# turtle-robotics/sea-current

Measured on AMD Instinct MI355X. Metric: plans/sec (batched start-goal, 1024^2 grid), higher is better.
Workload: dtype int32; 1 GPU; 1024x1024 random-obstacle grids (salt20, one grid and one query block per step), EDT + A*, 1024 batched queries per GPU and step, 10 steps = 10240 queries per library call; queries_per_launch=10240, map=salt20, queries_per_gpu=1024, queries_total=1024, lmax=4096, parallelism=query-sharded x1, contexts_in_flight=2, steps_per_call=10, hw_queues=4

## Files before the change

### sea-current_amd/csrc/astar.hip

```cpp
#include "sc_internal.h"
#include <stdlib.h>

#define NBUCKET 32
#define ASTAR_CQ_THROUGHPUT 1024
#define ASTAR_RU_THROUGHPUT 4
#define ASTAR_CQ_LATENCY 2048
#define ASTAR_RU_LATENCY 8
#define E_RUN (1u << 18)
#define E_START (4u << 13 | 3u << 16)
#define RUNK 8

struct astar_args {
    const uint8_t* moves;
    const int32_t* d2;
    int W, H;
    int32_t rmin;
    const int32_t* start;
    const int32_t* goal;
    const int32_t* qgrid;
    const int32_t* order;
    const int32_t* nq_dev;
    int nq;
    int Lmax;
    int32_t* path;
    int32_t* len;
    int32_t* cost;
    int32_t* status;
    void* g;
    uint32_t* closed;
    uint32_t* buckets;
    int cap;
    int32_t* expanded;
    int32_t* counter;
    int32_t* ovf_list;
    int32_t* ovf_count;
    int32_t* ovf_sticky;
    int nstat;
    int lazy;
    int tw, bw;
    size_t gcells, bwords;
};

__device__ __forceinline__ int octile(int x, int y, int gx, int gy) {
    int dx = abs(x - gx), dy = abs(y - gy);
    return 10 * max(dx, dy) + 4 * min(dx, dy);
}

__device__ __forceinline__ uint32_t gix(int x, int y, int tw) {
    return ((((uint32_t)(y >> 2) * (uint32_t)tw + (uint32_t)(x >> 2)) << 4) | ((uint32_t)(y & 3) << 2)) | (uint32_t)(x & 3);
}
__device__ __forceinline__ uint32_t gix8(int x, int y, int tw8) {
    return ((((uint32_t)(y >> 3) * (uint32_t)tw8 + (uint32_t)(x >> 3)) << 6) | ((uint32_t)(y & 7) << 3)) | (uint32_t)(x & 7);
}
template <typename GT> __device__ __forceinline__ uint32_t gidx(int x, int y, int tw);
template <> __device__ __forceinline__ uint32_t gidx<uint32_t>(int x, int y, int tw) { return gix(x, y, tw); }
template <> __device__ __forceinline__ uint32_t gidx<uint8_t>(int x, int y, int tw) { return gix8(x, y, tw); }
__device__ __forceinline__ uint32_t cix(int x, int y, int bw) {
    return (((uint32_t)(y >> 4) * (uint32_t)bw + (uint32_t)(x >> 5)) << 4) | (uint32_t)(y & 15);
}

template <typename T>
__device__ __forceinline__ T g_load(const T* p) {
    return __hip_atomic_load(p, __ATOMIC_RELAXED, __HIP_MEMORY_SCOPE_AGENT);
}

__device__ __forceinline__ uint32_t prune_always(int d) {
    const unsigned long long T = 0x75B6D9EA34C851A2ull;
    return (uint32_t)(T >> (8 * d)) & 0xFFu;
}

__device__ __forceinline__ uint32_t entry_pack(int x, int y, int d, uint32_t pmv) {
    const int e0 = (int)((0x6476u >> (4 * (d & 3))) & 7u), e1 = (int)((0x7554u >> (4 * (d & 3))) & 7u);
    const uint32_t side = d < 4 ? (((pmv >> e0) & 1u) | (((pmv >> e1) & 1u) << 1)) : 0u;
    return (uint32_t)y << 19 | side << 16 | (uint32_t)d << 13 | (uint32_t)x;
}
__device__ __forceinline__ uint32_t entry_prune(uint32_t e) {
    const int d = (int)((e >> 13) & 7u);
    uint32_t prune = prune_always(d);
    const int k0 = d < 2 ? 3 : 0, k1 = d < 2 ? 2 : 1;
    const int e0 = (int)((0x6476u >> (4 * (d & 3))) & 7u), e1 = (int)((0x7554u >> (4 * (d & 3))) & 7u);
    if ((e >> 16) & 1u) prune |= (1u << k0) | (1u << e0);
    if ((e >> 17) & 1u) prune |= (1u << k1) | (1u << e1);
    if (e & E_RUN) prune |= 1u << d;
    return (e & 0x3E000u) == E_START ? 0u : prune;
}
// ... 67 lines not shown
}

__device__ __forceinline__ uint32_t bcast_group8(uint32_t v) {
    const uint32_t q = (uint32_t)__builtin_amdgcn_update_dpp(0, (int)v, 0x00 , 0xF, 0xF, false);
    const uint32_t r = (uint32_t)__builtin_amdgcn_update_dpp(0, (int)q, 0x114 , 0xF, 0xF, false);
    return q | r;
}

#define HQ 256
#define ASTAR_SPIN_LIMIT (1 << 20)
template <typename GT, bool DUAL, int CQ, int REFILL_UNROLL>
__device__ __forceinline__ void astar_query(const astar_args& a, const int q, const int slot) {
    constexpr int REFILL = CQ / 2;
    __shared__ uint32_t qe[CQ + 64];
    __shared__ int s_head[NBUCKET];
    __shared__ int s_tail[NBUCKET];
    __shared__ uint32_t nd_xy[64];
    __shared__ uint32_t nd_mv[64];
    __shared__ uint16_t succ[512];
    __shared__ uint8_t prune_tbl[64];
    __shared__ uint32_t dup_tbl[DUAL ? 1024 + 64 : 1];
    __shared__ uint2 hq_rec[DUAL ? HQ + 64 : 1];
    __shared__ int hq_tail, hq_head, hq_clean, hq_stop, hq_ovf, hq_fcur, hq_found, hq_flush;
    constexpr int SCOPE = DUAL ? __HIP_MEMORY_SCOPE_WORKGROUP : __HIP_MEMORY_SCOPE_WAVEFRONT;
    const int lane = threadIdx.x & 63;
    const int wv = DUAL ? __builtin_amdgcn_readfirstlane((int)(threadIdx.x >> 6)) : 0;
    const int W = a.W, H = a.H;
    const size_t cells = (size_t)W * H;
    const int s = a.start[q], t = a.goal[q];
    int32_t* path = a.path + (size_t)q * a.Lmax;

    int out_st = SC_Q_OK, out_len = 0, out_cost = -1, nexp = 0, npop = 0, kcyc = 0, nstep = 0;
    const size_t grid_off = a.qgrid ? (size_t)a.qgrid[q] * cells : 0;
    const uint8_t* const mvs = a.moves + grid_off;
    const bool bad = s < 0 || t < 0 || (size_t)s >= cells || (size_t)t >= cells || a.d2[grid_off + s] < a.rmin || a.d2[grid_off + t] < a.rmin;
    if (bad) out_st = SC_Q_BAD_ENDPOINT;
    else if (s == t) {
        if (lane == 0 && wv == 0) path[0] = s;
        out_len = 1; out_cost = 0; nexp = 1;
    } else {
    const int tw = a.tw, bw = a.bw;
    GT* g = static_cast<GT*>(a.g) + (size_t)slot * a.gcells;
    uint32_t* cl = a.closed + (size_t)slot * a.bwords;
    uint32_t* bk = a.buckets + (size_t)slot * NBUCKET * a.cap;
    const int cap = a.cap, capm = a.cap - 1;
    const int sx = s % W, sy = s / W, gx = t % W, gy = t / W;
    const int ddx[8] = {1, -1, 0, 0, 1, -1, 1, -1};
    const int ddy[8] = {0, 0, 1, -1, 1, 1, -1, -1};

    {
        uint4* p = reinterpret_cast<uint4*>(cl);
        const size_t n4 = a.bwords >> 2;
        for (size_t i = DUAL ? threadIdx.x : lane; i < n4; i += DUAL ? 128 : 64) p[i] = make_uint4(0, 0, 0, 0);
    }
    __builtin_amdgcn_wave_barrier();
    if (wv == 0 && lane < NBUCKET) { s_head[lane] = 0; s_tail[lane] = 0; }
    if (wv == 0) prune_tbl[lane] = (uint8_t)entry_prune((uint32_t)lane << 13);
    if (DUAL)
        for (int i = threadIdx.x; i < 1024 + 64; i += 128) dup_tbl[i] = 0xFFFFFFFFu;
    int fcur = octile(sx, sy, gx, gy);
    if (wv == 0 && lane == 0) {
        qe[0] = (uint32_t)sy << 19 | E_START | (uint32_t)sx;
        hq_tail = 0; hq_head = 0; hq_clean = 0; hq_stop = 0; hq_ovf = 0; hq_fcur = fcur; hq_found = 0; hq_flush = 0;
    }
    asm volatile("s_waitcnt vmcnt(0)" ::: "memory");
    wave_lds_sync();
    if (DUAL) __syncthreads();
    int lh = 0, lt = 1;

    bool found = false, ovf = false;
    const unsigned long long t_begin = __builtin_amdgcn_s_memtime();
    int steps_left = (int)(8 * cells + 1024 < 0x7FFFFFFF ? 8 * cells + 1024 : 0x7FFFFFFF);

    const int mdx = (int)((0x2252u >> (2 * (lane & 7))) & 3u) - 1;
    const int mdy = (int)((0x0A25u >> (2 * (lane & 7))) & 3u) - 1;
    const uint32_t mw = (lane & 7) < 4 ? 10u : 14u;
    const int moff = mdy * W + mdx;

    auto push_entry = [&](const bool act, const uint32_t ne, const int df) {
        const bool same = act && df == 0;
        const unsigned long long m0 = __ballot(same);
        bool spill = false;
        if (m0) {
            const int cnt = __popcll(m0);
            if (__builtin_expect(lt - lh + cnt <= CQ, 1)) {
                if (same) {
                    const int rank = __builtin_amdgcn_mbcnt_hi((uint32_t)(m0 >> 32), __builtin_amdgcn_mbcnt_lo((uint32_t)m0, 0u));
                    qe[(lt + rank) & (CQ - 1)] = ne;
                }
                lt += cnt;
            } else spill = true;
        }
        if (act && (df != 0 || spill)) {
            const int bb = (fcur + df) & 31;
            const int pos = __hip_atomic_fetch_add(&s_tail[bb], 1, __ATOMIC_RELAXED, SCOPE);
            if (__builtin_expect(pos - __hip_atomic_load(&s_head[bb], __ATOMIC_RELAXED, SCOPE) >= cap, 0)) ovf = true;
            else bk[(size_t)bb * cap + (pos & capm)] = ne;
        }
        lt = __builtin_amdgcn_readfirstlane(lt);
    };
    int hq_tl = 0, hq_hd = 0;
    auto hand_over = [&](const bool rec, const int hx, const int hy, const uint32_t hm, const uint32_t hp) {
        const unsigned long long wm = __ballot(rec);
        if (wm) {
            const int cnt = __popcll(wm);
            int waited = 0;
            while (__builtin_expect(hq_tl + cnt - hq_hd > HQ, 0)) {
                hq_hd = __builtin_amdgcn_readfirstlane(__hip_atomic_load(&hq_head, __ATOMIC_RELAXED, SCOPE));
                if (hq_tl + cnt - hq_hd > HQ) {
                    __builtin_amdgcn_s_sleep(1);
// ... 127 lines not shown
                const int n = min(tl - hd, REFILL);
                for (int base = lane; base < n; base += 64 * REFILL_UNROLL) {
                    uint32_t chunk[REFILL_UNROLL];
#pragma unroll
                    for (int k = 0; k < REFILL_UNROLL; ++k)
                        if (base + 64 * k < n) chunk[k] = bq[(hd + base + 64 * k) & capm];
#pragma unroll
                    for (int k = 0; k < REFILL_UNROLL; ++k)
                        if (base + 64 * k < n) qe[(lt + base + 64 * k) & (CQ - 1)] = chunk[k];
                }
                lt += n;
                if (lane == 0) __hip_atomic_store(&s_head[b], hd + n, __ATOMIC_RELAXED, SCOPE);
                wave_lds_sync();
            }
            const int n = min(64, lt - lh);
            npop += n; ++nstep;
            if (DUAL && n <= 16) {
                const int kl = n <= 4 ? 3 : n <= 8 ? 2 : n <= 16 ? 1 : 0, KL = 1 << kl, GL = 2 * KL;
                const int sub = lane >> (kl + 1), j = (lane >> kl) & 1, k = lane & (KL - 1);
                const bool valid = sub < n;
                const uint32_t e_raw = qe[(lh + sub) & (CQ - 1)];
                const uint32_t e = valid ? e_raw : 0u;
                lh += n;
                const int x = e & 0x1FFF, y = e >> 19;
                const uint32_t bit = 1u << (x & 31);
                const int dxg = gx - x, dyg = gy - y, adx = abs(dxg), ady = abs(dyg);
                const int dD = 4 + ((dxg < 0 ? 1 : 0) | (dyg < 0 ? 2 : 0));
                const int dS = adx > ady ? (dxg < 0 ? 1 : 0) : (dyg < 0 ? 3 : 2);
                const uint32_t bD = adx >= 1 && ady >= 1 ? 1u << dD : 0u, bS = adx != ady ? 1u << dS : 0u;
                const int d = j ? dS : dD;
                const bool has = valid && (j ? bS : bD) != 0u;
                const int lgeom = j ? abs(adx - ady) : min(adx, ady);
                const int ddx_ = (int)((0x2252u >> (2 * d)) & 3u) - 1, ddy_ = (int)((0x0A25u >> (2 * d)) & 3u) - 1;
                const uint8_t* const addr = mvs + (y * W + x) + (has ? min(k, lgeom - 1) : 0) * (ddy_ * W + ddx_);
                const bool head = valid && j == 0 && k == 0;
                uint32_t old, byte;
                uint32_t* const wa = &cl[cix(x, y, bw)];
                pop_loads_issue(addr, wa, byte, old);
                const uint32_t prune = prune_tbl[(e >> 13) & 63u];
                const int dup = dup_settle(head, x, y, e);
                pop_loads_wait(byte, old);
                const bool link = has && k < lgeom && ((byte >> d) & 1u) && (k > 0 || !((prune >> d) & 1u));
                const unsigned long long lm = __ballot(link);
                const uint32_t grp = (uint32_t)(lm >> (lane & ~(KL - 1))) & ((1u << KL) - 1u);
                const int run = __ffs((int)~grp) - 1;
                const uint32_t ne = entry_pack(x + (k + 1) * ddx_, y + (k + 1) * ddy_, d, byte) | (k + 1 < run ? E_RUN : 0u);
                const bool won1 = head && dup == 0 && !(old & bit);
                masked_or_noret(wa, won1 ? bit : 0u);
                const unsigned long long wm1 = __ballot(won1);
                const bool act = ((wm1 >> (lane & ~(GL - 1))) & 1ull) && k < run;
                {
                    const unsigned long long ma = __ballot(act);
                    if (ma) {
                        const int c = __popcll(ma);
                        if (__builtin_expect(lt - lh + c <= CQ, 1)) {
                            qe[act ? ((lt + (int)__builtin_amdgcn_mbcnt_hi((uint32_t)(ma >> 32), __builtin_amdgcn_mbcnt_lo((uint32_t)ma, 0u))) & (CQ - 1)) : CQ + lane] = ne;
                            lt += c;
                        } else push_entry(act, ne, 0);
                    }
                }
                hand_over(won1, x, y, (byte & ~prune) & ~(bD | bS), byte);
                nexp += __popcll(wm1);
            } else if (!DUAL && n <= 8) {
                const int sub = lane >> 3, d = lane & 7;
                const bool valid = sub < n;
                const uint32_t e = valid ? qe[(lh + sub) & (CQ - 1)] : 0u;
                lh += n;
                const int x = e & 0x1FFF, y = e >> 19;
                const uint32_t bit = 1u << (x & 31);
                uint32_t old = 0, pmv;
                const int hc = octile(x, y, gx, gy);
                const int nx = x + mdx, ny = y + mdy;
                const int df = (int)mw + octile(nx, ny, gx, gy) - hc;
                const int adx = abs(gx - x), ady = abs(gy - y);
                const int lgeom = d >= 4 ? min(adx, ady) : abs(adx - ady);
                const int lmax = valid && df == 0 ? min(RUNK, lgeom) : 1;
                const uint8_t* const cell = mvs + (y * W + x);
                const uint8_t* ra[RUNK - 1];
                uint32_t rm[RUNK - 1];
#pragma unroll
                for (int k = 1; k < RUNK; ++k) ra[k - 1] = cell + min(k, lmax - 1) * moff;
                pop_run_issue(ra, cell, &cl[cix(x, y, bw)], valid && d == 0 ? bit : 0u, rm, pmv, old);
                const uint32_t prune = prune_tbl[(e >> 13) & 63u];
                pop_run_wait_loads(rm, pmv, old);
                const bool cand = valid && (((pmv & ~prune) >> d) & 1u);
                int run = cand ? 1 : 0;
#pragma unroll
                for (int k = 1; k < RUNK; ++k)
                    if (run == k && k < lmax && ((rm[k - 1] >> d) & 1u)) run = k + 1;
                const uint32_t ne = entry_pack(nx, ny, d, pmv) | (run > 1 ? E_RUN : 0u);
                atomic_wait(old);
                old = bcast_group8(old);
                const bool won = valid && !(old & bit);
                push_entry(won && cand, ne, df);
#pragma unroll
                for (int k = 2; k <= RUNK; ++k) {
                    if (__ballot(won && run >= k) == 0) break;
                    push_entry(won && run >= k, entry_pack(x + k * mdx, y + k * mdy, d, rm[k - 2]) | (run > k ? E_RUN : 0u), 0);
                }
                nexp += __popcll(__ballot(won && d == 0));
                if (__ballot(won && x == gx && y == gy)) found = true;
                if (won && d == 0) g[gidx<GT>(x, y, tw)] = (GT)(fcur - hc);
            } else if (DUAL) {
                const bool valid = lane < n;
                const uint32_t e_raw = qe[(lh + lane) & (CQ - 1)];
                const uint32_t e = valid ? e_raw : 0u;
                lh += n;
                const int x = e & 0x1FFF, y = e >> 19;
                const uint32_t bit = 1u << (x & 31);
                uint32_t old, pmv;
                uint32_t* const wa = &cl[cix(x, y, bw)];
                pop_loads_issue(mvs + (y * W + x), wa, pmv, old);
                const int dup = dup_settle(valid, x, y, e);
                const uint32_t prune = prune_tbl[(e >> 13) & 63u];
                const int dxg = gx - x, dyg = gy - y, adx = abs(dxg), ady = abs(dyg);
                const int dD = 4 + ((dxg < 0 ? 1 : 0) | (dyg < 0 ? 2 : 0));
                const int dS = adx > ady ? (dxg < 0 ? 1 : 0) : (dyg < 0 ? 3 : 2);
                const uint32_t bD = adx >= 1 && ady >= 1 ? 1u << dD : 0u, bS = adx != ady ? 1u << dS : 0u;
                const int nxD = x + (dxg < 0 ? -1 : 1), nyD = y + (dyg < 0 ? -1 : 1);
                const int nxS = x + (adx > ady ? (dxg < 0 ? -1 : 1) : 0), nyS = y + (adx > ady ? 0 : (dyg < 0 ? -1 : 1));
                pop_loads_wait(pmv, old);
                const uint32_t cand = valid ? (pmv & ~prune) : 0u;
                const uint32_t neD = (uint32_t)nyD << 19 | (uint32_t)dD << 13 | (uint32_t)nxD;
                const uint32_t neS = entry_pack(nxS, nyS, dS, pmv);
                const bool won = valid && dup == 0 && !(old & bit);
                masked_or_noret(wa, won ? bit : 0u);
                {
                    const bool pD = won && (cand & bD), pS = won && (cand & bS);
                    const unsigned long long mD = __ballot(pD), mS = __ballot(pS);
                    const int cD = __popcll(mD), c2 = cD + __popcll(mS);
                    if (c2) {
                        if (__builtin_expect(lt - lh + c2 <= CQ, 1)) {
                            qe[pD ? ((lt + (int)__builtin_amdgcn_mbcnt_hi((uint32_t)(mD >> 32), __builtin_amdgcn_mbcnt_lo((uint32_t)mD, 0u))) & (CQ - 1)) : CQ + lane] = neD;
                            qe[pS ? ((lt + cD + (int)__builtin_amdgcn_mbcnt_hi((uint32_t)(mS >> 32), __builtin_amdgcn_mbcnt_lo((uint32_t)mS, 0u))) & (CQ - 1)) : CQ + lane] = neS;
                            lt += c2;
                        } else {
                            push_entry(pD, neD, 0);
                            push_entry(pS, neS, 0);
                        }
                    }
                }
                nexp += __popcll(hand_over(won, x, y, cand & ~(bD | bS), pmv));
            } else {
                const bool valid = lane < n;
                const uint32_t e = valid ? qe[(lh + lane) & (CQ - 1)] : 0u;
                lh += n;
                const int x = e & 0x1FFF, y = e >> 19;
                const uint32_t bit = 1u << (x & 31);
                uint32_t old = 0, pmv;
                pop_pair_issue(mvs + (y * W + x), &cl[cix(x, y, bw)], valid ? bit : 0u, pmv, old);
                const uint32_t prune = prune_tbl[(e >> 13) & 63u];
                const int hc = octile(x, y, gx, gy);
                pop_pair_wait_load(pmv, old);
                uint32_t mv = valid ? (pmv & ~prune) : 0u;
                nd_xy[lane] = (uint32_t)y << 16 | (uint32_t)x;
                nd_mv[lane] = pmv;
                const uint32_t cnt = (uint32_t)__popc(mv);
                int base = 0, total = 0;
#pragma unroll
                for (int bb = 0; bb < 4; ++bb) {
                    const unsigned long long m = __ballot((cnt >> bb) & 1u);
                    base += (int)__builtin_amdgcn_mbcnt_hi((uint32_t)(m >> 32), __builtin_amdgcn_mbcnt_lo((uint32_t)m, 0u)) << bb;
                    total += __popcll(m) << bb;
                }
                while (mv) {
                    const int dd = __ffs((int)mv) - 1;
                    mv &= mv - 1;
                    succ[base++] = (uint16_t)(lane << 3 | dd);
                }
                wave_lds_sync();
                bool won = false;
                for (int j0 = 0; j0 < total; j0 += 64) {
                    const bool act = j0 + lane < total;
                    const uint32_t sd = act ? succ[j0 + lane] : 0u;
                    const int par = (int)(sd >> 3), d = (int)(sd & 7u);
                    const uint32_t xy = nd_xy[par], pmvp = nd_mv[par];
                    const int px = xy & 0xFFFF, py = xy >> 16;
                    const int ddx_ = (int)((0x2252u >> (2 * d)) & 3u) - 1, ddy_ = (int)((0x0A25u >> (2 * d)) & 3u) - 1;
                    const int nx = px + ddx_, ny = py + ddy_;
                    const int df = (d < 4 ? 10 : 14) + octile(nx, ny, gx, gy) - octile(px, py, gx, gy);
                    const uint8_t* ra[RUNK - 1];
#pragma unroll
                    for (int k = 1; k < RUNK; ++k) ra[k - 1] = mvs + (py * W + px);
                    (void)ra;
                    if (j0 == 0) {
                        atomic_wait(old);
                        won = valid && !(old & bit);
                        nexp += __popcll(__ballot(won));
                        if (__ballot(won && x == gx && y == gy)) found = true;
                        nd_mv[lane] = pmv | (won ? 0x100u : 0u);
                        wave_lds_sync();
                    }
                    const bool go = act && ((nd_mv[par] >> 8) & 1u);
                    push_entry(go, entry_pack(nx, ny, d, pmvp), df);
                }
                if (total == 0) {
                    atomic_wait(old);
                    won = valid && !(old & bit);
                    nexp += __popcll(__ballot(won));
                    if (__ballot(won && x == gx && y == gy)) found = true;
                }
                if (won) g[gidx<GT>(x, y, tw)] = (GT)(fcur - hc);
            }
            lt = __builtin_amdgcn_readfirstlane(lt);
            lh = __builtin_amdgcn_readfirstlane(lh);
            nexp = __builtin_amdgcn_readfirstlane(nexp);
            found = __builtin_amdgcn_readfirstlane((int)found) != 0;
            wave_lds_sync();
            if (--steps_left < 0) ovf = true;
            if (__builtin_expect(DUAL ? steps_left < 0 : __ballot(ovf) != 0, 0)) break;
        }
        if (DUAL) {
            if (a.lazy && lane == 0) __hip_atomic_store(&hq_flush, hq_tl, __ATOMIC_RELAXED, SCOPE);
            for (int waited = 0; __builtin_amdgcn_readfirstlane(__hip_atomic_load(&hq_clean, __ATOMIC_RELAXED, SCOPE)) != hq_tl;) {
                __builtin_amdgcn_s_sleep(1);
                if (++waited > ASTAR_SPIN_LIMIT) { ovf = true; break; }
// ... 12 lines not shown
        fcur += 1 + (__ffs((int)rot) - 1);
        if (DUAL && lane == 0) __hip_atomic_store(&hq_fcur, fcur, __ATOMIC_RELAXED, SCOPE);
    }
    if (DUAL && lane == 0) __hip_atomic_store(&hq_stop, 1, __ATOMIC_RELAXED, SCOPE);
    }
    if (DUAL) __syncthreads();

    const bool overflow = __ballot(ovf) != 0;
    if (overflow) {
        if (lane == 0 && wv == 0) {
            const int i = atomicAdd(a.ovf_count, 1);
            a.ovf_list[i] = q;
            *a.ovf_sticky = 1;
        }
        out_st = SC_Q_RING_OVERFLOW;
    } else if (!found) {
        out_st = SC_Q_NO_PATH;
    } else {
        asm volatile("s_waitcnt vmcnt(0)" ::: "memory");
        const int Lmax = a.Lmax;
        int cx = gx, cy = gy, L = 1;
        uint32_t gc = (uint32_t)fcur;
        if (lane == 0) path[Lmax - 1] = t;
        bool broken = false;
        const int wox = lane % 7 - 3, woy = lane / 7 - 3;
        const int md = lane & 7;
        const int mdx_ = (int)((0x2252u >> (2 * md)) & 3u) - 1, mdy_ = (int)((0x0A25u >> (2 * md)) & 3u) - 1;
        const uint32_t mw_ = md < 4 ? 10u : 14u;
        while (!broken && (cx != sx || cy != sy)) {
            uint32_t info = 0u, gw = 0u;
            {
                const int nx = cx + wox, ny = cy + woy;
                if (lane < 49 && nx >= 0 && ny >= 0 && nx < W && ny < H) {
                    const uint32_t mvb = mvs[ny * W + nx];
                    const uint32_t cw = g_load(&cl[cix(nx, ny, bw)]);
                    gw = (uint32_t)g_load(&g[gidx<GT>(nx, ny, tw)]);
                    info = mvb | ((cw >> (nx & 31)) & 1u) << 8;
                }
            }
            int ox = 0, oy = 0;
            for (int k = 0; k < 3 && !broken && (cx != sx || cy != sy); ++k) {
                const int src = (oy - mdy_ + 3) * 7 + (ox - mdx_ + 3);
                const uint32_t ni = (uint32_t)__shfl((int)info, src, 64), ng = (uint32_t)__shfl((int)gw, src, 64);
                const bool ok = lane < 8 && ((ni >> md) & 1u) && ((ni >> 8) & 1u) && (GT)ng == (GT)(gc - mw_);
                const unsigned long long m = __ballot(ok);
                if (!m) broken = true;
                else {
                    const int d = __ffsll((long long)m) - 1;
                    cx -= ddx[d]; cy -= ddy[d];
                    ox -= ddx[d]; oy -= ddy[d];
                    gc -= (d < 4 ? 10u : 14u);
                    ++L;
                    if (lane == 0 && L <= Lmax) path[Lmax - L] = cy * W + cx;
                }
            }
        }
        if (broken) out_st = SC_Q_NO_PATH;
        else if (L > Lmax) { out_st = SC_Q_TRUNCATED; out_len = L; out_cost = fcur; }
        else {
            const int shift = Lmax - L;
            if (shift > 0) {
                __builtin_amdgcn_fence(__ATOMIC_RELEASE, "workgroup");
                for (int i = 0; i < L; i += 64) {
                    int v = 0;
                    if (i + lane < L) v = __hip_atomic_load(&path[shift + i + lane], __ATOMIC_RELAXED, __HIP_MEMORY_SCOPE_AGENT);
                    if (i + lane < L) path[i + lane] = v;
                    __builtin_amdgcn_fence(__ATOMIC_RELEASE, "workgroup");
                }
            }
            out_len = L; out_cost = fcur;
        }
    }
    kcyc = (int)((__builtin_amdgcn_s_memtime() - t_begin) >> 10);
    }
    if (lane == 0 && wv == 0) {
        a.status[q] = out_st; a.len[q] = out_len; a.cost[q] = out_cost;
        a.expanded[q] = nexp; a.expanded[a.nstat + q] = npop; a.expanded[2 * a.nstat + q] = kcyc; a.expanded[3 * a.nstat + q] = nstep;
    }
}

template <typename GT>
__global__ void __launch_bounds__(64) astar_kernel(astar_args a) {
    const int nq = a.nq_dev ? *a.nq_dev : a.nq;
    for (;;) {
        const int qi = __builtin_amdgcn_readfirstlane(atomicAdd(a.counter, 1)) >> 6;
        if (qi >= nq) break;
        astar_query<GT, false, ASTAR_CQ_THROUGHPUT, ASTAR_RU_THROUGHPUT>(a, a.order ? a.order[qi] : qi, (int)blockIdx.x);
    }
}

template <typename GT, int CQ, int RU>
__global__ void __launch_bounds__(128) astar_kernel_dual(astar_args a) {
    __shared__ int s_qi;
    const int nq = a.nq_dev ? *a.nq_dev : a.nq;
    for (;;) {
        if (threadIdx.x == 0) s_qi = atomicAdd(a.counter, 64) >> 6;
        __syncthreads();
        const int qi = __builtin_amdgcn_readfirstlane(s_qi);
        __syncthreads();
        if (qi >= nq) break;
        astar_query<GT, true, CQ, RU>(a, a.order ? a.order[qi] : qi, (int)blockIdx.x);
        __syncthreads();
    }
}

__global__ void __launch_bounds__(1024) astar_prep_kernel(const int32_t* __restrict__ start, const int32_t* __restrict__ goal, int Q, int W,
                                                          int H, int32_t* __restrict__ order, int32_t* __restrict__ ctr) {
    __shared__ int hist[1024];
    __shared__ int scan[1024];
    const int tid = threadIdx.x;
    if (tid < 4) ctr[tid] = 0;
    if (!order) return;
    hist[tid] = 0;
    __syncthreads();
    const int hmax = 14 * max(W, H) + 1;
// ... 31 lines not shown
    int per_cu = 0, dev = ctx->device;
    hipDeviceProp_t prop;
    if (hipOccupancyMaxActiveBlocksPerMultiprocessor(&per_cu, astar_kernel<uint8_t>, 64, 0) != hipSuccess || per_cu <= 0) per_cu = 8;
    if (hipGetDeviceProperties(&prop, dev) != hipSuccess || prop.multiProcessorCount <= 0) prop.multiProcessorCount = 256;
    int w = per_cu * prop.multiProcessorCount;
    if (const char* e = getenv("SC_ASTAR_WAVES")) { const int v = atoi(e); if (v > 0) w = v; }
    ctx->astar_waves = w;
    return w;
}
static int astar_resident_dual(sc_ctx* ctx, bool latency) {
    int& cached = latency ? ctx->astar_dual_lat : ctx->astar_dual;
    if (cached >= 0) return cached;
    int per_cu = 0, n = 0;
    hipDeviceProp_t prop;
    const hipError_t e_ = latency ? hipOccupancyMaxActiveBlocksPerMultiprocessor(&per_cu, astar_kernel_dual<uint8_t, ASTAR_CQ_LATENCY, ASTAR_RU_LATENCY>, 128, 0)
                                  : hipOccupancyMaxActiveBlocksPerMultiprocessor(&per_cu, astar_kernel_dual<uint8_t, ASTAR_CQ_THROUGHPUT, ASTAR_RU_THROUGHPUT>, 128, 0);
    if (e_ == hipSuccess && per_cu > 0 && hipGetDeviceProperties(&prop, ctx->device) == hipSuccess && prop.multiProcessorCount > 0)
        n = per_cu * prop.multiProcessorCount;
    if (const char* e = getenv("SC_ASTAR_DUAL")) { const int v = atoi(e); if (v == 0) n = 0; else if (v > 1 && v < n) n = v; }
    if (latency) { if (const char* e = getenv("SC_ASTAR_LATENCY")) { if (atoi(e) == 0) n = 0; } }
    cached = n;
    return n;
}

static int astar_run(sc_ctx* ctx, const int32_t* d2, int G, const int32_t* qgrid, int W, int H, int32_t r2, const int32_t* start,
                     const int32_t* goal, int Q, int Lmax, int32_t* path, int32_t* len, int32_t* cost,
                     int32_t* status, bool full_g = false) {
    const size_t cells = (size_t)W * H;
    const int tw = full_g ? (W + 3) >> 2 : (W + 7) >> 3, bw = (W + 31) >> 5;
    const size_t gcells = full_g ? (size_t)tw * ((H + 3) >> 2) * 16 : (size_t)tw * ((H + 7) >> 3) * 64;
    const size_t gsz = full_g ? 4 : 1;
    const size_t bwords = (size_t)bw * ((H + 15) >> 4) * 16;
    const int32_t rmin = r2 > 1 ? r2 : 1;
    int r = sc_scratch_reserve(ctx, &ctx->moves, cells * (size_t)G);
    if (r != SC_OK) return r;
    r = sc_launch_moves(ctx, d2, W, H * G, H, r2, (uint8_t*)ctx->moves.p);
    if (r != SC_OK) return r;
    r = sc_scratch_reserve(ctx, &ctx->qstats, (size_t)Q * 6 * sizeof(int32_t));
    if (r != SC_OK) return r;
    int32_t* expanded = (int32_t*)ctx->qstats.p;
    int32_t* order = expanded + 4 * (size_t)Q;
    int32_t* ovf_list = order + Q;
    ctx->last_Q = Q;
    int cap = ctx->astar_cap;
    if (const char* e = getenv("SC_ASTAR_CAP")) { const int v = atoi(e); if (v >= 1024 && (v & (v - 1)) == 0) cap = v; }
    if (cells > ((size_t)1 << 21)) {
        int want = 1 << 15;
        while (want < 64 * (W > H ? W : H)) want <<= 1;
        if (cap < want) cap = want;
    }
    const size_t per_slot = gcells * gsz + bwords * 4 + (size_t)NBUCKET * cap * 4;
    size_t slots = ctx->astar_slot_budget / per_slot;
    const size_t rlat = (size_t)astar_resident_dual(ctx, true);
    const bool latency = !full_g && rlat > 0 && (size_t)Q <= rlat && (size_t)Q <= slots;
    const size_t rdual = latency ? rlat : (size_t)astar_resident_dual(ctx, false);
    const bool dual = !full_g && rdual > 0;
    const size_t resident = dual ? rdual : (size_t)astar_resident_waves(ctx);
    if (slots > resident) slots = resident;
    if (slots > (size_t)Q) slots = Q;
    if (slots < 1) slots = 1;
    auto ring_slots = [](size_t n) { return n > 16 ? n : (size_t)16; };
    if (slots * gcells * gsz > ctx->gslots.bytes || slots * bwords * 4 > ctx->closed.bytes || ring_slots(slots) * NBUCKET * (size_t)cap * 4 > ctx->buckets.bytes) {
        size_t free_b = 0, total_b = 0;
        if (hipMemGetInfo(&free_b, &total_b) == hipSuccess) {
            const size_t avail = (size_t)(0.9 * (double)(free_b + ctx->gslots.bytes + ctx->closed.bytes + ctx->buckets.bytes));
            while (slots > 1 && slots * (gcells * gsz + bwords * 4) + ring_slots(slots) * NBUCKET * (size_t)cap * 4 > avail) slots = (slots + 1) / 2;
        }
    }
    for (;;) {
        r = sc_scratch_reserve(ctx, &ctx->gslots, slots * gcells * gsz);
        if (r == SC_OK) r = sc_scratch_reserve(ctx, &ctx->closed, slots * bwords * 4);
        if (r == SC_OK) r = sc_scratch_reserve(ctx, &ctx->buckets, ring_slots(slots) * NBUCKET * (size_t)cap * 4);
        if (r == SC_OK) break;
        if (r != SC_ERR_NOMEM || slots <= 1) return r;
        (void)hipGetLastError();
        slots = (slots + 1) / 2;
    }
    if (!ctx->actr.p) {
        r = sc_scratch_reserve(ctx, &ctx->actr, 16 * sizeof(int32_t));
        if (r != SC_OK) return r;
        SC_HIP(ctx, hipMemsetAsync(ctx->actr.p, 0, 16 * sizeof(int32_t), ctx->stream));
    }
    int32_t* ctr = (int32_t*)ctx->actr.p;
    ctx->status_armed = true;

    const bool sorted = (size_t)Q > slots;
    int tk = sc_time_begin(ctx, SC_K_ASTAR);
    hipLaunchKernelGGL(astar_prep_kernel, dim3(1), dim3(1024), 0, ctx->stream, start, goal, Q, W, H, sorted ? order : (int32_t*)nullptr, ctr);
    astar_args a{(const uint8_t*)ctx->moves.p, d2, W, H, rmin, start, goal, qgrid, sorted ? order : nullptr, nullptr, Q, Lmax, path, len,
                 cost, status, ctx->gslots.p, (uint32_t*)ctx->closed.p, (uint32_t*)ctx->buckets.p, cap, expanded, ctr,
                 ovf_list, ctr + 1, ctx->status + SC_ST_ASTAR_OVERFLOW, Q, (dual && (size_t)Q > slots) ? 1 : 0, tw, bw, gcells, bwords};
    if (full_g) hipLaunchKernelGGL(astar_kernel<uint32_t>, dim3((unsigned)slots), dim3(64), 0, ctx->stream, a);
    else if (dual && latency && (size_t)Q <= slots)
        hipLaunchKernelGGL((astar_kernel_dual<uint8_t, ASTAR_CQ_LATENCY, ASTAR_RU_LATENCY>), dim3((unsigned)slots), dim3(128), 0, ctx->stream, a);
    else if (dual)
        hipLaunchKernelGGL((astar_kernel_dual<uint8_t, ASTAR_CQ_THROUGHPUT, ASTAR_RU_THROUGHPUT>), dim3((unsigned)slots), dim3(128), 0, ctx->stream, a);
    else hipLaunchKernelGGL(astar_kernel<uint8_t>, dim3((unsigned)slots), dim3(64), 0, ctx->stream, a);
    {
        const size_t rslots = slots >= 16 ? slots / 16 : 1;
        const int rcap = cap * 16;
        astar_args b = a;
        b.order = ovf_list; b.nq_dev = ctr + 1; b.nq = 0; b.cap = rcap; b.counter = ctr + 2;
        b.ovf_list = order; b.ovf_count = ctr + 3;
        if (full_g) hipLaunchKernelGGL(astar_kernel<uint32_t>, dim3((unsigned)rslots), dim3(64), 0, ctx->stream, b);
        else hipLaunchKernelGGL(astar_kernel<uint8_t>, dim3((unsigned)rslots), dim3(64), 0, ctx->stream, b);
    }
    sc_time_end(ctx, tk);
    SC_HIP(ctx, hipGetLastError());
    return SC_OK;
}

extern "C" int sc_astar_batch(sc_ctx* ctx, const int32_t* d2, int W, int H, int32_t r2_clear,
                              const int32_t* start, const int32_t* goal, int Q, int Lmax,
                              int32_t* path, int32_t* len, int32_t* cost, int32_t* status) {
    if (!ctx || !d2 || !start || !goal || !path || !len || !cost || !status || W <= 0 || H <= 0 || Q < 0 ||
        Lmax <= 0 || W > SC_MAX_DIM || H > SC_MAX_DIM)
        return SC_ERR_INVALID;
    if (Q == 0) return SC_OK;
    SC_HIP(ctx, hipSetDevice(ctx->device));
    return astar_run(ctx, d2, 1, nullptr, W, H, r2_clear, start, goal, Q, Lmax, path, len, cost, status);
}

extern "C" int sc_astar_batch_multi(sc_ctx* ctx, const int32_t* d2, int G, const int32_t* qgrid, int W, int H, int32_t r2_clear,
                                    const int32_t* start, const int32_t* goal, int Q, int Lmax,
// ... 59 lines not shown
```

### sea-current_amd/csrc/moves.hip

```cpp
#include "sc_internal.h"

__global__ void __launch_bounds__(256)
moves_kernel(const int32_t* __restrict__ d2, int W, int Hall, int H, int32_t rmin, uint8_t* __restrict__ moves) {
    const int x = blockIdx.x * 256 + threadIdx.x;
    const int yall = blockIdx.y;
    if (x >= W) return;
    const int y = yall % H;
    const int32_t* r1 = d2 + (size_t)yall * W;
    bool t[3][3];
#pragma unroll
    for (int j = -1; j <= 1; ++j)
#pragma unroll
        for (int i = -1; i <= 1; ++i) {
            int xx = x + i, yy = y + j;
            t[j + 1][i + 1] = xx >= 0 && xx < W && yy >= 0 && yy < H && r1[(ptrdiff_t)j * W + xx] >= rmin;
        }
    uint32_t m = 0;
    if (t[1][1]) {
        m |= (uint32_t)t[1][2] << 0;
        m |= (uint32_t)t[1][0] << 1;
        m |= (uint32_t)t[2][1] << 2;
        m |= (uint32_t)t[0][1] << 3;
        m |= (uint32_t)(t[2][2] && t[1][2] && t[2][1]) << 4;
        m |= (uint32_t)(t[2][0] && t[1][0] && t[2][1]) << 5;
// ... 52 lines not shown
        const int32_t* r = r1 + (ptrdiff_t)(j - 1) * W;
        const int4 v = *reinterpret_cast<const int4*>(r + x);
        const int32_t l = x > 0 ? r[x - 1] : 0, q = x + 4 < W ? r[x + 4] : 0;
        t[j] = (uint32_t)(l >= rmin) | (uint32_t)(v.x >= rmin) << 1 | (uint32_t)(v.y >= rmin) << 2 | (uint32_t)(v.z >= rmin) << 3 |
               (uint32_t)(v.w >= rmin) << 4 | (uint32_t)(q >= rmin) << 5;
    }
#pragma unroll
    for (int k = 0; k < 4; ++k) {
        uint32_t out = 0;
#pragma unroll
        for (int i = 0; i < 4; ++i) {
            const uint32_t a = t[k] >> i, c = t[k + 1] >> i, b = t[k + 2] >> i;
            uint32_t m = 0;
            if (c & 2u) {
                const uint32_t E = (c >> 2) & 1u, Wt = c & 1u, S = (b >> 1) & 1u, N = (a >> 1) & 1u;
                m = E | Wt << 1 | S << 2 | N << 3 | (((b >> 2) & 1u) & E & S) << 4 | ((b & 1u) & Wt & S) << 5 | (((a >> 2) & 1u) & E & N) << 6 |
                    ((a & 1u) & Wt & N) << 7;
            }
            out |= m << (8 * i);
        }
        *reinterpret_cast<uint32_t*>(moves + (size_t)(yall0 + k) * W + x) = out;
    }
}

int sc_launch_moves(sc_ctx* ctx, const int32_t* d2, int W, int Hall, int H, int32_t r2, uint8_t* moves) {
    int32_t rmin = r2 > 1 ? r2 : 1;
    int tk = sc_time_begin(ctx, SC_K_MOVES);
    if (W % 4 == 0 && H % 4 == 0 && ((uintptr_t)d2 & 15) == 0 && ((uintptr_t)moves & 3) == 0)
        hipLaunchKernelGGL(moves4x4_kernel, dim3((W / 4 + 255) / 256, Hall / 4), dim3(256), 0, ctx->stream, d2, W, Hall, H, rmin, moves);
    else if (W % 4 == 0 && ((uintptr_t)d2 & 15) == 0 && ((uintptr_t)moves & 3) == 0)
        hipLaunchKernelGGL(moves4_kernel, dim3((W / 4 + 255) / 256, Hall), dim3(256), 0, ctx->stream, d2, W, Hall, H, rmin, moves);
    else
        hipLaunchKernelGGL(moves_kernel, dim3((W + 255) / 256, Hall), dim3(256), 0, ctx->stream, d2, W, Hall, H, rmin, moves);
    sc_time_end(ctx, tk);
    SC_HIP(ctx, hipGetLastError());
    return SC_OK;
}

extern "C" int sc_moves_i32_u8(sc_ctx* ctx, const int32_t* d2, int W, int H, int32_t r2_clear, uint8_t* moves) {
    if (!ctx || !d2 || !moves || W <= 0 || H <= 0 || W > SC_MAX_DIM || H > SC_MAX_DIM) return SC_ERR_INVALID;
    SC_HIP(ctx, hipSetDevice(ctx->device));
    return sc_launch_moves(ctx, d2, W, H, H, r2_clear, moves);
}

__host__ __device__ static inline int64_t isqrt64(int64_t v) {
    int64_t r = (int64_t)sqrt((double)v);
    while (r * r > v) --r;
    while ((r + 1) * (r + 1) <= v) ++r;
    return r;
}

__global__ void __launch_bounds__(256)
clearance_penalty_kernel(const int32_t* __restrict__ d2, size_t n, int32_t thr, int32_t r2_soft, int64_t s10, int pen_max,
                         uint8_t* __restrict__ pen) {
    const size_t i = (size_t)blockIdx.x * 256 + threadIdx.x;
    if (i >= n) return;
    const int32_t d = d2[i];
    uint8_t p = 0;
    if (d >= thr && d < r2_soft) p = (uint8_t)(((int64_t)pen_max * (s10 - isqrt64(100ll * d))) / s10);
    pen[i] = p;
}

extern "C" int sc_clearance_penalty_u8(sc_ctx* ctx, const int32_t* d2, int W, int H, int batch, int32_t r2_clear, int32_t r2_soft,
                                       int pen_max, uint8_t* pen) {
    if (!ctx || !d2 || !pen || W <= 0 || H <= 0 || W > SC_MAX_DIM || H > SC_MAX_DIM || batch <= 0 || pen_max < 0 || pen_max > 255 ||
        r2_soft < 1)
// ... 26 lines not shown
```

### sea-current_amd/csrc/sc_internal.h

```cpp
#pragma once
#include <hip/hip_runtime.h>
#include <math.h>
#include <stdint.h>
#include <stdio.h>
#include <string.h>

#include <set>
#include <vector>

#include "../../include/sea_current_hip.h"

struct sc_scratch {
    void* p = nullptr;
    size_t bytes = 0;
    sc_scratch() = default;
    sc_scratch(const sc_scratch&) = delete;
    sc_scratch& operator=(const sc_scratch&) = delete;
    ~sc_scratch() { if (p) (void)hipFree(p); }
};

static inline size_t al256(size_t b) { return (b + 255) & ~(size_t)255; }

enum sc_status_word {
    SC_ST_ASTAR_OVERFLOW,
// ... 95 lines not shown
class __attribute__((visibility("hidden"))) sc_stage {
  public:
    explicit sc_stage(sc_ctx* ctx) : ctx_(ctx) {}
    int in(const void* src, size_t bytes) {
        const int i = slot(bytes);
        if (src && bytes) up_.push_back({i, const_cast<void*>(src), bytes});
        return i;
    }
    int out(void* dst, size_t bytes) {
        const int i = slot(bytes);
        back(i, dst, bytes);
        return i;
    }
    void back(int i, void* dst, size_t bytes) {
        if (dst && bytes) down_.push_back({i, dst, bytes});
    }
    int upload();
    template <class T> T* dev(int i) const { return (T*)((char*)ctx_->host_stage.p + off_[i]); }
    int finish(int r);

  private:
    struct copy { int slot; void* host; size_t bytes; };
    int slot(size_t bytes) {
        off_.push_back(end_);
        end_ += al256(bytes ? bytes : 1);
        return (int)off_.size() - 1;
    }
    sc_ctx* ctx_;
    size_t end_ = 0;
    std::vector<size_t> off_;
    std::vector<copy> up_, down_;
};

int sc_time_begin(sc_ctx* ctx, int kid);
void sc_time_end(sc_ctx* ctx, int token);
int sc_time_chain(sc_ctx* ctx, int token, int kid);

int sc_launch_edt(sc_ctx* ctx, const uint8_t* occ, int W, int H, int batch, int32_t* d2);
int sc_launch_moves(sc_ctx* ctx, const int32_t* d2, int W, int Hall, int H, int32_t r2, uint8_t* moves);
int sc_launch_arclength(sc_ctx* ctx, const float* ctrl, int S, int nsub, float* cum, float* seg_len, const int32_t* S_dev);
int sc_launch_resample(sc_ctx* ctx, const float* ctrl, const float* cum, const float* arclength, const int32_t* seg_off, int B, int S,
                       int nsub, float* profile_pos, const int32_t* prof_off, int nudge, float* pts, float* tpar, int32_t* seg,
                       float* curvature, int32_t* status, const int32_t* S_dev);
struct sc_speed_frame {
    const int32_t* d2;
    int W, H;
    float x_min, y_min, res_x, res_y;
};
static inline bool sc_frame_ok(const sc_speed_frame& fr) {
    return fr.W >= 1 && fr.W <= SC_MAX_DIM && fr.H >= 1 && fr.H <= SC_MAX_DIM && isfinite(fr.x_min) && isfinite(fr.y_min) &&
           isfinite(fr.res_x) && fr.res_x > 0.f && isfinite(fr.res_y) && fr.res_y > 0.f;
}
int sc_launch_speed_limits(sc_ctx* ctx, const float* ctrl, const float* cum, const int32_t* seg_off, const float* arclength,
                           const int32_t* status, int P, int nsub, int N, int J, const double* limits, const double* dyn,
                           const sc_speed_frame& fr, int ns_bound, double* vlo, double* vhi, double* vhi_copy, float* min_clear,
                           int32_t* status_out);
int sc_speed_args_ok(int J, const double* dyn, const sc_speed_frame& fr);
int sc_speed_dyn_ok(const double* dyn, int P);
int sc_curve_grid_ok(const sc_speed_frame& fr, int32_t r2_clear);
int sc_launch_curve_clear(sc_ctx* ctx, const float* ctrl_in, float* ctrl_out, const int32_t* seg_off, const int32_t* status, int P,
                          const sc_speed_frame& fr, int32_t r2_clear, int max_level, uint8_t* level, int32_t* rounds, int32_t* leg_min,
                          int32_t* status_out);
int sc_launch_toppra_sample_packed(sc_ctx* ctx, int P, int dof, int N, const double* p0, const double* p1, const double* v0,
                                   const double* v1, const double* x, const double* t, double dt, const int32_t* offsets,
                                   const int32_t* plen, const int32_t* skip, float* pos, float* vel, float* acc, double* times);

int sc_allow_big_lds(sc_ctx* ctx, const void* kernel, int bytes);

int sc_stream_wait(sc_ctx* ctx);
void sc_edt_open_mode_update(sc_ctx* ctx, int32_t seen, int32_t still);

#ifdef __HIPCC__
// ... 21 lines not shown
```

Before: 721,700 plans/s.

## Store A* move bytes in 8x8 tiled layout with column-major tiles

```diff
diff --git a/sea-current_amd/csrc/astar.hip b/sea-current_amd/csrc/astar.hip
--- a/sea-current_amd/csrc/astar.hip
+++ b/sea-current_amd/csrc/astar.hip
@@ -39,6 +39,8 @@
     int lazy;
     int tw, bw;
     size_t gcells, bwords;
+    uint32_t mstep;
+    size_t mcells;
 };
 
 __device__ __forceinline__ int octile(int x, int y, int gx, int gy) {
@@ -48,9 +50,6 @@
 
 __device__ __forceinline__ uint32_t gix(int x, int y, int tw) {
     return ((((uint32_t)(y >> 2) * (uint32_t)tw + (uint32_t)(x >> 2)) << 4) | ((uint32_t)(y & 3) << 2)) | (uint32_t)(x & 3);
-}
-__device__ __forceinline__ uint32_t gix8(int x, int y, int tw8) {
-    return ((((uint32_t)(y >> 3) * (uint32_t)tw8 + (uint32_t)(x >> 3)) << 6) | ((uint32_t)(y & 7) << 3)) | (uint32_t)(x & 7);
 }
 template <typename GT> __device__ __forceinline__ uint32_t gidx(int x, int y, int tw);
 template <> __device__ __forceinline__ uint32_t gidx<uint32_t>(int x, int y, int tw) { return gix(x, y, tw); }
@@ -184,7 +183,7 @@
 
     int out_st = SC_Q_OK, out_len = 0, out_cost = -1, nexp = 0, npop = 0, kcyc = 0, nstep = 0;
     const size_t grid_off = a.qgrid ? (size_t)a.qgrid[q] * cells : 0;
-    const uint8_t* const mvs = a.moves + grid_off;
+    const uint8_t* const mvs = a.moves + (a.qgrid ? (size_t)a.qgrid[q] * a.mcells : 0);
     const bool bad = s < 0 || t < 0 || (size_t)s >= cells || (size_t)t >= cells || a.d2[grid_off + s] < a.rmin || a.d2[grid_off + t] < a.rmin;
     if (bad) out_st = SC_Q_BAD_ENDPOINT;
     else if (s == t) {
@@ -192,6 +191,7 @@
         out_len = 1; out_cost = 0; nexp = 1;
     } else {
     const int tw = a.tw, bw = a.bw;
+    const uint32_t mstep = a.mstep;
     GT* g = static_cast<GT*>(a.g) + (size_t)slot * a.gcells;
     uint32_t* cl = a.closed + (size_t)slot * a.bwords;
     uint32_t* bk = a.buckets + (size_t)slot * NBUCKET * a.cap;
@@ -227,7 +227,6 @@
     const int mdx = (int)((0x2252u >> (2 * (lane & 7))) & 3u) - 1;
     const int mdy = (int)((0x0A25u >> (2 * (lane & 7))) & 3u) - 1;
     const uint32_t mw = (lane & 7) < 4 ? 10u : 14u;
-    const int moff = mdy * W + mdx;
 
     auto push_entry = [&](const bool act, const uint32_t ne, const int df) {
         const bool same = act && df == 0;
@@ -421,7 +420,8 @@
                 const bool has = valid && (j ? bS : bD) != 0u;
                 const int lgeom = j ? abs(adx - ady) : min(adx, ady);
                 const int ddx_ = (int)((0x2252u >> (2 * d)) & 3u) - 1, ddy_ = (int)((0x0A25u >> (2 * d)) & 3u) - 1;
-                const uint8_t* const addr = mvs + (y * W + x) + (has ? min(k, lgeom - 1) : 0) * (ddy_ * W + ddx_);
+                const int kc = has ? min(k, lgeom - 1) : 0;
+                const uint8_t* const addr = mvs + mvix(x + kc * ddx_, y + kc * ddy_, mstep);
                 const bool head = valid && j == 0 && k == 0;
                 uint32_t old, byte;
                 uint32_t* const wa = &cl[cix(x, y, bw)];
@@ -464,11 +464,11 @@
                 const int adx = abs(gx - x), ady = abs(gy - y);
                 const int lgeom = d >= 4 ? min(adx, ady) : abs(adx - ady);
                 const int lmax = valid && df == 0 ? min(RUNK, lgeom) : 1;
-                const uint8_t* const cell = mvs + (y * W + x);
+                const uint8_t* const cell = mvs + mvix(x, y, mstep);
                 const uint8_t* ra[RUNK - 1];
                 uint32_t rm[RUNK - 1];
 #pragma unroll
-                for (int k = 1; k < RUNK; ++k) ra[k - 1] = cell + min(k, lmax - 1) * moff;
+                for (int k = 1; k < RUNK; ++k) ra[k - 1] = mvs + mvix(x + min(k, lmax - 1) * mdx, y + min(k, lmax - 1) * mdy, mstep);
                 pop_run_issue(ra, cell, &cl[cix(x, y, bw)], valid && d == 0 ? bit : 0u, rm, pmv, old);
                 const uint32_t prune = prune_tbl[(e >> 13) & 63u];
                 pop_run_wait_loads(rm, pmv, old);
@@ -499,7 +499,7 @@
                 const uint32_t bit = 1u << (x & 31);
                 uint32_t old, pmv;
                 uint32_t* const wa = &cl[cix(x, y, bw)];
-                pop_loads_issue(mvs + (y * W + x), wa, pmv, old);
+                pop_loads_issue(mvs + mvix(x, y, mstep), wa, pmv, old);
                 const int dup = dup_settle(valid, x, y, e);
                 const uint32_t prune = prune_tbl[(e >> 13) & 63u];
                 const int dxg = gx - x, dyg = gy - y, adx = abs(dxg), ady = abs(dyg);
@@ -537,7 +537,7 @@
                 const int x = e & 0x1FFF, y = e >> 19;
                 const uint32_t bit = 1u << (x & 31);
                 uint32_t old = 0, pmv;
-                pop_pair_issue(mvs + (y * W + x), &cl[cix(x, y, bw)], valid ? bit : 0u, pmv, old);
+                pop_pair_issue(mvs + mvix(x, y, mstep), &cl[cix(x, y, bw)], valid ? bit : 0u, pmv, old);
                 const uint32_t prune = prune_tbl[(e >> 13) & 63u];
                 const int hc = octile(x, y, gx, gy);
                 pop_pair_wait_load(pmv, old);
@@ -570,7 +570,7 @@
                     const int df = (d < 4 ? 10 : 14) + octile(nx, ny, gx, gy) - octile(px, py, gx, gy);
                     const uint8_t* ra[RUNK - 1];
 #pragma unroll
-                    for (int k = 1; k < RUNK; ++k) ra[k - 1] = mvs + (py * W + px);
+                    for (int k = 1; k < RUNK; ++k) ra[k - 1] = mvs + mvix(px, py, mstep);
                     (void)ra;
                     if (j0 == 0) {
                         atomic_wait(old);
@@ -649,7 +649,7 @@
             {
                 const int nx = cx + wox, ny = cy + woy;
                 if (lane < 49 && nx >= 0 && ny >= 0 && nx < W && ny < H) {
-                    const uint32_t mvb = mvs[ny * W + nx];
+                    const uint32_t mvb = mvs[mvix(nx, ny, mstep)];
                     const uint32_t cw = g_load(&cl[cix(nx, ny, bw)]);
                     gw = (uint32_t)g_load(&g[gidx<GT>(nx, ny, tw)]);
                     info = mvb | ((cw >> (nx & 31)) & 1u) << 8;
@@ -697,7 +697,7 @@
 }
 
 template <typename GT>
-__global__ void __launch_bounds__(64) astar_kernel(astar_args a) {
+__global__ void __launch_bounds__(64, 5) astar_kernel(astar_args a) {
     const int nq = a.nq_dev ? *a.nq_dev : a.nq;
     for (;;) {
         const int qi = __builtin_amdgcn_readfirstlane(atomicAdd(a.counter, 1)) >> 6;
@@ -795,9 +795,10 @@
     const size_t gsz = full_g ? 4 : 1;
     const size_t bwords = (size_t)bw * ((H + 15) >> 4) * 16;
     const int32_t rmin = r2 > 1 ? r2 : 1;
-    int r = sc_scratch_reserve(ctx, &ctx->moves, cells * (size_t)G);
+    const size_t mcells = sc_moves_cells(W, H);
+    int r = sc_scratch_reserve(ctx, &ctx->moves, mcells * (size_t)G);
     if (r != SC_OK) return r;
-    r = sc_launch_moves(ctx, d2, W, H * G, H, r2, (uint8_t*)ctx->moves.p);
+    r = sc_launch_moves_tiled(ctx, d2, W, H, G, r2, (uint8_t*)ctx->moves.p);
     if (r != SC_OK) return r;
     r = sc_scratch_reserve(ctx, &ctx->qstats, (size_t)Q * 6 * sizeof(int32_t));
     if (r != SC_OK) return r;
@@ -852,7 +853,7 @@
     hipLaunchKernelGGL(astar_prep_kernel, dim3(1), dim3(1024), 0, ctx->stream, start, goal, Q, W, H, sorted ? order : (int32_t*)nullptr, ctr);
     astar_args a{(const uint8_t*)ctx->moves.p, d2, W, H, rmin, start, goal, qgrid, sorted ? order : nullptr, nullptr, Q, Lmax, path, len,
                  cost, status, ctx->gslots.p, (uint32_t*)ctx->closed.p, (uint32_t*)ctx->buckets.p, cap, expanded, ctr,
-                 ovf_list, ctr + 1, ctx->status + SC_ST_ASTAR_OVERFLOW, Q, (dual && (size_t)Q > slots) ? 1 : 0, tw, bw, gcells, bwords};
+                 ovf_list, ctr + 1, ctx->status + SC_ST_ASTAR_OVERFLOW, Q, (dual && (size_t)Q > slots) ? 1 : 0, tw, bw, gcells, bwords, sc_moves_step(W), mcells};
     if (full_g) hipLaunchKernelGGL(astar_kernel<uint32_t>, dim3((unsigned)slots), dim3(64), 0, ctx->stream, a);
     else if (dual && latency && (size_t)Q <= slots)
         hipLaunchKernelGGL((astar_kernel_dual<uint8_t, ASTAR_CQ_LATENCY, ASTAR_RU_LATENCY>), dim3((unsigned)slots), dim3(128), 0, ctx->stream, a);
diff --git a/sea-current_amd/csrc/moves.hip b/sea-current_amd/csrc/moves.hip
--- a/sea-current_amd/csrc/moves.hip
+++ b/sea-current_amd/csrc/moves.hip
@@ -108,6 +108,101 @@
         hipLaunchKernelGGL(moves4_kernel, dim3((W / 4 + 255) / 256, Hall), dim3(256), 0, ctx->stream, d2, W, Hall, H, rmin, moves);
     else
         hipLaunchKernelGGL(moves_kernel, dim3((W + 255) / 256, Hall), dim3(256), 0, ctx->stream, d2, W, Hall, H, rmin, moves);
+    sc_time_end(ctx, tk);
+    SC_HIP(ctx, hipGetLastError());
+    return SC_OK;
+}
+
+__global__ void __launch_bounds__(256)
+moves4x4_tiled_kernel(const int32_t* __restrict__ d2, int W, int H, int G, int mtw, uint32_t mstep, size_t mcells, int32_t rmin, uint8_t* __restrict__ moves) {
+    constexpr int TXT = 1 << (MT_LX - 2), TYT = 1 << (MT_LY - 2), TPT = TXT * TYT;
+    const int t = threadIdx.x;
+    const int tile_x = blockIdx.x * (256 / TPT) + t / TPT;
+    if (tile_x >= mtw) return;
+    const int x = (tile_x << MT_LX) + 4 * (t % TXT);
+    const int y0 = ((int)blockIdx.y << MT_LY) + 4 * ((t / TXT) % TYT);
+    const bool inside = x < W && y0 < H;
+    for (int g = blockIdx.z; g < G; g += gridDim.z) {
+        const int32_t* r1 = d2 + (size_t)g * W * H + (size_t)y0 * W;
+        uint32_t tr[6];
+#pragma unroll
+        for (int j = 0; j < 6; ++j) {
+            const int yy = y0 + j - 1;
+            tr[j] = 0u;
+            if (!inside || yy < 0 || yy >= H) continue;
+            const int32_t* r = r1 + (ptrdiff_t)(j - 1) * W;
+            const int4 v = *reinterpret_cast<const int4*>(r + x);
+            const int32_t l = x > 0 ? r[x - 1] : 0, q = x + 4 < W ? r[x + 4] : 0;
+            tr[j] = (uint32_t)(l >= rmin) | (uint32_t)(v.x >= rmin) << 1 | (uint32_t)(v.y >= rmin) << 2 | (uint32_t)(v.z >= rmin) << 3 |
+                    (uint32_t)(v.w >= rmin) << 4 | (uint32_t)(q >= rmin) << 5;
+        }
+        uint8_t* mg = moves + (size_t)g * mcells;
+        uint32_t col[4] = {0u, 0u, 0u, 0u};
+#pragma unroll
+        for (int k = 0; k < 4; ++k) {
+#pragma unroll
+            for (int i = 0; i < 4; ++i) {
+                const uint32_t a = tr[k] >> i, c = tr[k + 1] >> i, b = tr[k + 2] >> i;
+                uint32_t m = 0;
+                if (c & 2u) {
+                    const uint32_t E = (c >> 2) & 1u, Wt = c & 1u, S = (b >> 1) & 1u, N = (a >> 1) & 1u;
+                    m = E | Wt << 1 | S << 2 | N << 3 | (((b >> 2) & 1u) & E & S) << 4 | ((b & 1u) & Wt & S) << 5 | (((a >> 2) & 1u) & E & N) << 6 |
+                        ((a & 1u) & Wt & N) << 7;
+                }
+                col[i] |= m << (8 * k);
+            }
+        }
+#pragma unroll
+        for (int i = 0; i < 4; ++i) *reinterpret_cast<uint32_t*>(mg + mvix(x + i, y0, mstep)) = col[i];
+    }
+}
+
+__global__ void __launch_bounds__(256)
+moves_tiled_kernel(const int32_t* __restrict__ d2, int W, int H, int G, int mtw, size_t mcells, int32_t rmin, uint8_t* __restrict__ moves) {
+    const size_t i = (size_t)blockIdx.x * 256 + threadIdx.x;
+    if (i >= mcells) return;
+    const uint32_t tile = (uint32_t)(i >> (MT_LX + MT_LY));
+    const int x = (int)((tile % (uint32_t)mtw) << MT_LX) + (int)((i >> MT_LY) & ((1 << MT_LX) - 1));
+    const int y = (int)((tile / (uint32_t)mtw) << MT_LY) + (int)(i & ((1 << MT_LY) - 1));
+    const bool inside = x < W && y < H;
+    for (int g = blockIdx.y; g < G; g += gridDim.y) {
+        uint32_t m = 0;
+        if (inside) {
+            const int32_t* r1 = d2 + (size_t)g * W * H + (size_t)y * W;
+            bool t[3][3];
+#pragma unroll
+            for (int j = -1; j <= 1; ++j)
+#pragma unroll
+                for (int ii = -1; ii <= 1; ++ii) {
+                    const int xx = x + ii, yy = y + j;
+                    t[j + 1][ii + 1] = xx >= 0 && xx < W && yy >= 0 && yy < H && r1[(ptrdiff_t)j * W + xx] >= rmin;
+                }
+            if (t[1][1]) {
+                m |= (uint32_t)t[1][2] << 0;
+                m |= (uint32_t)t[1][0] << 1;
+                m |= (uint32_t)t[2][1] << 2;
+                m |= (uint32_t)t[0][1] << 3;
+                m |= (uint32_t)(t[2][2] && t[1][2] && t[2][1]) << 4;
+                m |= (uint32_t)(t[2][0] && t[1][0] && t[2][1]) << 5;
+                m |= (uint32_t)(t[0][2] && t[1][2] && t[0][1]) << 6;
+                m |= (uint32_t)(t[0][0] && t[1][0] && t[0][1]) << 7;
+            }
+        }
+        moves[(size_t)g * mcells + i] = (uint8_t)m;
+    }
+}
+
+int sc_launch_moves_tiled(sc_ctx* ctx, const int32_t* d2, int W, int H, int G, int32_t r2, uint8_t* moves) {
+    const int32_t rmin = r2 > 1 ? r2 : 1;
+    const int mtw = sc_moves_tw(W), mth = (H + (1 << MT_LY) - 1) >> MT_LY;
+    const size_t mcells = sc_moves_cells(W, H);
+    const unsigned gz = (unsigned)(G < 65535 ? G : 65535);
+    int tk = sc_time_begin(ctx, SC_K_MOVES);
+    if (W % 4 == 0 && H % 4 == 0 && ((uintptr_t)d2 & 15) == 0 && ((uintptr_t)moves & 3) == 0) {
+        constexpr int TILES = 256 >> (MT_LX + MT_LY - 4);
+        hipLaunchKernelGGL(moves4x4_tiled_kernel, dim3((mtw + TILES - 1) / TILES, mth, gz), dim3(256), 0, ctx->stream, d2, W, H, G, mtw, sc_moves_step(W), mcells, rmin, moves);
+    } else
+        hipLaunchKernelGGL(moves_tiled_kernel, dim3((unsigned)((mcells + 255) / 256), gz), dim3(256), 0, ctx->stream, d2, W, H, G, mtw, mcells, rmin, moves);
     sc_time_end(ctx, tk);
     SC_HIP(ctx, hipGetLastError());
     return SC_OK;
diff --git a/sea-current_amd/csrc/sc_internal.h b/sea-current_amd/csrc/sc_internal.h
--- a/sea-current_amd/csrc/sc_internal.h
+++ b/sea-current_amd/csrc/sc_internal.h
@@ -151,12 +151,36 @@
     std::vector<copy> up_, down_;
 };
 
+__host__ __device__ static inline uint32_t gix8(int x, int y, int tw8) {
+    return ((((uint32_t)(y >> 3) * (uint32_t)tw8 + (uint32_t)(x >> 3)) << 6) | ((uint32_t)(y & 7) << 3)) | (uint32_t)(x & 7);
+}
+#ifndef MT_LX
+#define MT_LX 3
+#endif
+#ifndef MT_LY
+#define MT_LY 3
+#endif
+static_assert(MT_LX >= 2 && MT_LX <= 5 && MT_LY >= 2 && MT_LY <= 5, "tiles of whole 4 x 4 blocks, at most 32 x 32 cells");
+__host__ __device__ static inline uint32_t mvix(int x, int y, uint32_t mstep) {
+#if defined(__HIP_DEVICE_COMPILE__)
+    return __umul24((uint32_t)(y >> MT_LY), mstep) + (uint32_t)y + ((uint32_t)x << MT_LY);
+#else
+    return (uint32_t)(y >> MT_LY) * mstep + (uint32_t)y + ((uint32_t)x << MT_LY);
+#endif
+}
+static inline int sc_moves_tw(int W) { return (W + (1 << MT_LX) - 1) >> MT_LX; }
+static inline uint32_t sc_moves_step(int W) { return ((uint32_t)sc_moves_tw(W) << (MT_LX + MT_LY)) - (1u << MT_LY); }
+static inline size_t sc_moves_cells(int W, int H) {
+    return ((size_t)sc_moves_tw(W) * (size_t)((H + (1 << MT_LY) - 1) >> MT_LY)) << (MT_LX + MT_LY);
+}
+
 int sc_time_begin(sc_ctx* ctx, int kid);
 void sc_time_end(sc_ctx* ctx, int token);
 int sc_time_chain(sc_ctx* ctx, int token, int kid);
 
 int sc_launch_edt(sc_ctx* ctx, const uint8_t* occ, int W, int H, int batch, int32_t* d2);
 int sc_launch_moves(sc_ctx* ctx, const int32_t* d2, int W, int Hall, int H, int32_t r2, uint8_t* moves);
+int sc_launch_moves_tiled(sc_ctx* ctx, const int32_t* d2, int W, int H, int G, int32_t r2, uint8_t* moves);
 int sc_launch_arclength(sc_ctx* ctx, const float* ctrl, int S, int nsub, float* cum, float* seg_len, const int32_t* S_dev);
 int sc_launch_resample(sc_ctx* ctx, const float* ctrl, const float* cum, const float* arclength, const int32_t* seg_off, int B, int S,
                        int nsub, float* profile_pos, const int32_t* prof_off, int nudge, float* pts, float* tpar, int32_t* seg,
```

Result: faster. 743,100 plans/s (median of 6 runs) (+3.0%).
